# PINTO0309/human-instance-segmentation

Hardware: AMD Instinct MI355X
Metric: ROI-masks/sec (fwd) + train step/s, B0 640×480×8-ROI, 1/2/4/8 MI355X (higher is better)
Workload: dtype bf16; 1 GPU; C2: B0 inference 640x480, batch 32/GPU x 8 ROIs/img, ROI 64x48, mask 128x96; global_batch=32, parallelism=dp1 (images sharded, model replicated, no collective), schedule=2-stream pipeline (UNet of step k+1 overlaps head of step k)

## Files before the change

human-instance-segmentation_amd/csrc/conv_common.h:

```cpp
#pragma once
#include "common.h"

namespace hiseg {

typedef __bf16 bf16x8_t __attribute__((ext_vector_type(8)));
typedef float floatx4 __attribute__((ext_vector_type(4)));

struct ConvArgs {
  hiseg_conv2d_desc d;
  int M;
  int Cin;
  int nK;
  int Hs, Ws;
  int kper;
  int ins_vec;
  float* ws;
  int abl = 0;
};

int conv_fast_try(const ConvArgs& a, hipStream_t s, int variant);
int conv_wide_try(const ConvArgs& a, hipStream_t s, int variant);
int conv_hw_try(const ConvArgs& a, hipStream_t s, int variant);
int conv_hwr_try(const ConvArgs& a, hipStream_t s, int variant);
int conv_hwt_try(const ConvArgs& a, hipStream_t s, int variant);
int conv_hwc_try(const ConvArgs& a, hipStream_t s, int variant);
int conv_pw_try(const ConvArgs& a, hipStream_t s, int variant);
int conv_small_try(const ConvArgs& a, hipStream_t s, int variant);
int conv_rows_try(const ConvArgs& a, hipStream_t s, int variant);
bool conv_pw_applies(const ConvArgs& a);
int conv_pw_gate_images(const ConvArgs& a);
bool conv_rows_form(const ConvArgs& a);
int conv_hwc_stats_tiles(const ConvArgs& a);
int conv_hwc_fused_variant(const ConvArgs& a, bool r3);
int conv_generic_launch(const ConvArgs& a, hipStream_t s, int splits, int* bco);
int splitk_plan(const ConvArgs& a);
long long splitk_bytes(const ConvArgs& a, int splits);

template <typename T>
__device__ __forceinline__ void load4(const void* base, long long idx, bool vec, int nvalid,
                                      float* v) {
  if (vec) {
    if constexpr (sizeof(T) == 4) {
      float4 q = *reinterpret_cast<const float4*>(reinterpret_cast<const float*>(base) + idx);
      v[0] = q.x; v[1] = q.y; v[2] = q.z; v[3] = q.w;
    } else {
      uint2 q = *reinterpret_cast<const uint2*>(reinterpret_cast<const uint16_t*>(base) + idx);
      v[0] = __uint_as_float(q.x << 16); v[1] = __uint_as_float(q.x & 0xffff0000u);
      v[2] = __uint_as_float(q.y << 16); v[3] = __uint_as_float(q.y & 0xffff0000u);
    }
  } else {
#pragma unroll
    for (int e = 0; e < 4; ++e) v[e] = (e < nvalid) ? Elem<T>::load(base, idx + e) : 0.f;
  }
}

template <typename T>
__device__ __forceinline__ void store4(void* base, long long idx, bool vec, int nvalid,
                                       const float* v) {
  if (vec) {
    if constexpr (sizeof(T) == 4) {
      *reinterpret_cast<float4*>(reinterpret_cast<float*>(base) + idx) =
          make_float4(v[0], v[1], v[2], v[3]);
    } else {
      uint2 q;
      q.x = f2bf2(v[0], v[1]);
      q.y = f2bf2(v[2], v[3]);
      *reinterpret_cast<uint2*>(reinterpret_cast<uint16_t*>(base) + idx) = q;
    }
  } else {
#pragma unroll
    for (int e = 0; e < 4; ++e)
      if (e < nvalid) Elem<T>::store(base, idx + e, v[e]);
  }
}

__device__ __forceinline__ int swz(int row, int c) { return row * 8 + (c ^ ((row >> 1) & 7)); }

__device__ __forceinline__ void out_site(const hiseg_conv2d_desc& d, int px, int co, long long& op, int& oc) {
  if (d.convT) {
    const int Cq = d.Cout >> 2;
    const int q = co / Cq;
    oc = co - q * Cq;
    const int x = px % d.Wo;
    const int t = px / d.Wo;
    const int y = t % d.Ho;
    const int n = t / d.Ho;
// ... 148 lines not shown
```

human-instance-segmentation_amd/csrc/conv_dispatch.cpp:

```cpp
#include <atomic>
#include <climits>
#include <cstdlib>
#include "conv_common.h"

using namespace hiseg;

static std::atomic<long long> g_conv_paths[HISEG_CONV_PATH_FAMILIES];
static thread_local int g_conv_last = -1;

static void conv_note_path(int family, int variant) {
  g_conv_paths[family].fetch_add(1);
  g_conv_last = family * 10000 + variant;
}

extern "C" int hiseg_conv2d_last_path(void) { return g_conv_last; }

extern "C" int hiseg_conv2d_path_stats(long long* counts, int n, int reset) {
  for (int i = 0; i < HISEG_CONV_PATH_FAMILIES; ++i) {
    const long long c = reset ? g_conv_paths[i].exchange(0) : g_conv_paths[i].load();
    if (counts && i < n) counts[i] = c;
  }
  return HISEG_CONV_PATH_FAMILIES;
}

// ... 240 lines not shown
  return HISEG_OK;
}

static int conv2d_impl(const hiseg_conv2d_desc* d, hiseg_stream_t stream, int variant) {
  HISEG_REQUIRE(d != nullptr, HISEG_ERR_BAD_ARG, "conv2d: null descriptor");
  HISEG_REQUIRE(d->dtype == HISEG_F32 || d->dtype == HISEG_BF16, HISEG_ERR_BAD_DTYPE, "conv2d: dtype %d", d->dtype);
  HISEG_REQUIRE(d->out_dtype == HISEG_F32 || d->out_dtype == HISEG_BF16, HISEG_ERR_BAD_DTYPE, "conv2d: out_dtype %d", d->out_dtype);
  HISEG_REQUIRE(d->srcA && d->weight && d->scale && d->shift && (d->out || d->head2_out), HISEG_ERR_BAD_ARG,
                "conv2d: null pointer");
#ifdef HISEG_DIAG
  const bool fused_variant = variant == 0 || (variant == 148 && d->a_gate);
#else
  const bool fused_variant = variant == 0;
#endif
  HISEG_REQUIRE(!has_fused_operands(d) ||
                    (fused_variant && !d->stats_partial && !d->bnb_partial && fused_operands_ok(d)),
                HISEG_ERR_BAD_ARG,
                "conv2d: px_scale / head2_out / a_gate / res_gate go with the automatic choice alone: px_scale or "
                "a_gate by itself, res_gate only beside head2_out");
  HISEG_REQUIRE(d->N > 0 && d->H > 0 && d->W > 0 && d->Ho > 0 && d->Wo > 0, HISEG_ERR_BAD_SHAPE, "conv2d: empty grid");
  HISEG_REQUIRE(d->KH > 0 && d->KW > 0 && d->stride > 0 && d->pad >= 0, HISEG_ERR_BAD_SHAPE, "conv2d: bad window");
  HISEG_REQUIRE(d->a_up == 1 || d->a_up == 2, HISEG_ERR_BAD_SHAPE, "conv2d: a_up must be 1 or 2");
  HISEG_REQUIRE(d->a_up == 1 || (d->H % 2 == 0 && d->W % 2 == 0), HISEG_ERR_BAD_SHAPE, "conv2d: upsampled grid must be even");
  HISEG_REQUIRE(d->Cb == 0 || d->srcB, HISEG_ERR_BAD_ARG, "conv2d: Cb > 0 needs srcB");
  HISEG_REQUIRE(d->Cout > 0 && d->Cout_pad >= d->Cout && d->Cout_pad % 16 == 0, HISEG_ERR_BAD_SHAPE,
                "conv2d: Cout %d Cout_pad %d (must be multiple of 16)", d->Cout, d->Cout_pad);
  const int kch = d->dtype == HISEG_BF16 ? 8 : 4;
  const int bk = 8 * kch;
  const int Cin = d->Ca + d->Cb;
  HISEG_REQUIRE(d->Ca > 0 && d->Ca % kch == 0 && d->Cb % kch == 0 && d->a_cstride % kch == 0 &&
                    d->a_coff % kch == 0 && (d->Cb == 0 || (d->b_cstride % kch == 0 && d->b_coff % kch == 0)),
                HISEG_ERR_BAD_SHAPE, "conv2d: input channels/strides must be multiples of %d", kch);
  HISEG_REQUIRE(d->K_pad % bk == 0 && d->K_pad >= d->KH * d->KW * Cin, HISEG_ERR_BAD_SHAPE,
                "conv2d: K_pad %d must be a multiple of %d and >= %d", d->K_pad, bk, d->KH * d->KW * Cin);
  HISEG_REQUIRE(al16(d->srcA) && al16(d->srcB) && al16(d->weight), HISEG_ERR_BAD_SHAPE, "conv2d: operands must be 16-B aligned");
  HISEG_REQUIRE(!d->convT || (d->KH == 1 && d->KW == 1 && d->stride == 1 && d->pad == 0 && d->Cout % 16 == 0 &&
                              d->Ho == d->H && d->Wo == d->W),
                HISEG_ERR_BAD_SHAPE, "conv2d: convT requires a 1x1 GEMM with Cout = 4*C, C %% 4 == 0");
  hipStream_t s = (hipStream_t)stream;
  if (d->stats_partial || d->bnb_partial) {
    HISEG_REQUIRE(variant == 0 || variant == 104 || variant == 107, HISEG_ERR_BAD_ARG,
                  "conv2d: stats_partial / bnb_partial with variant %d", variant);
    HISEG_REQUIRE(al16(d->out) && al16(d->scale) && al16(d->shift), HISEG_ERR_BAD_SHAPE, "conv2d: alignment");
    const ConvArgs a = conv_args(*d);
    HISEG_REQUIRE(conv_hwc_stats_tiles(a) > 0, HISEG_ERR_BAD_ARG,
                  "conv2d: stats_partial / bnb_partial set but the layer has no fused kernel (hiseg_conv2d_stats_tiles)");
    const int r = conv_take({&kFamilies[F_HWC], d->Cout % 128 == 0 ? 104 : 107}, a, s);
    HISEG_REQUIRE(r != 0, HISEG_ERR_BAD_ARG, "conv2d: the fused-statistics kernel declined the layer");
    return r < 0 ? r : HISEG_OK;
  }
  return conv_in_ranges(d, s, variant);
}

extern "C" int hiseg_conv2d_fwd(const hiseg_conv2d_desc* d, hiseg_stream_t stream) {
  return conv2d_impl(d, stream, 0);
}

extern "C" int hiseg_conv2d_fwd_variant(const hiseg_conv2d_desc* d, int variant, hiseg_stream_t stream) {
#ifndef HISEG_DIAG
  HISEG_REQUIRE(release_variant(variant), HISEG_ERR_BAD_ARG,
                "conv2d: variant %d is not a release variant (diagnostic kernels need a DIAG=1 build)", variant);
#endif
  return conv2d_impl(d, stream, variant);
}
```

human-instance-segmentation_amd/hiseg/_lib.py:

```python
from __future__ import annotations

import contextlib
import ctypes
import os

import torch

_HERE = os.path.dirname(os.path.abspath(__file__))
LIB_PATH = os.environ.get("HISEG_LIB", os.path.join(_HERE, "libhiseg.so"))

HISEG_F32 = 0
HISEG_BF16 = 1
HISEG_POST_F32, HISEG_POST_F16, HISEG_POST_F32_TO_F16 = 0, 2, 3
ACT_NONE, ACT_RELU, ACT_SIGMOID, ACT_SILU, ACT_GELU, ACT_SWISH = 0, 1, 2, 3, 4, 5


class ActCode(int):

    def __new__(cls, code: int, beta: float = 1.0):
        o = int.__new__(cls, code)
        o.beta = float(beta)
        return o

    def __repr__(self):
# ... 200 lines not shown

class GuidedPrepDesc(Desc):
    _fields_ = [("mask", c_void_p), ("mask_stride", c_ll), ("N", c_int), ("h", c_int), ("w", c_int), ("dtype", c_int),
                ("fgp_c", c_void_p), ("fgp_cstride", c_int), ("fgp_coff", c_int),
                ("fg_prob", c_void_p), ("factor", c_void_p)]


class GuidedAttnDesc(Desc):
    _fields_ = [("dtype", c_int), ("x", c_void_p), ("P", c_ll), ("C", c_int), ("hidden", c_int),
                ("w1t", c_void_p), ("b1", c_void_p), ("w2", c_void_p), ("b2", c_void_p),
                ("act", c_int), ("act_beta", c_float),
                ("factor", c_void_p), ("att", c_void_p), ("gate", c_void_p), ("w1_frag", c_void_p)]


class GuidedFinishDesc(Desc):
    _fields_ = [("dtype", c_int), ("z", c_void_p), ("N", c_int), ("h", c_int), ("w", c_int), ("C", c_int),
                ("w3", c_void_p), ("b3", c_void_p), ("mh", c_int), ("mw", c_int), ("logits", c_void_p),
                ("mask", c_void_p), ("mask_stride", c_ll),
                ("bg_fg_logits", c_void_p), ("fg_prob", c_void_p), ("mask_out", c_void_p), ("tn_logits", c_void_p)]


class HisegError(RuntimeError):
    """Raised when a libhiseg entry point returns a non-zero status."""


_lib = None
_load_error = None


def _declare(lib):
    P = c_void_p
    sigs = {
        "hiseg_version": ([], c_int),
        "hiseg_last_error_string": ([], ctypes.c_char_p),
        "hiseg_built_for_gfx950": ([], c_int),
        "hiseg_stream_create_cu_mask": ([ctypes.POINTER(ctypes.c_uint), c_int, ctypes.POINTER(c_void_p)], c_int),
        "hiseg_stream_destroy": ([P], c_int),
        "hiseg_comm_load": ([ctypes.c_char_p], c_int),
        "hiseg_comm_unique_id": ([P], c_int),
        "hiseg_comm_init": ([ctypes.POINTER(c_void_p), c_int, P, c_int, c_int], c_int),
        "hiseg_comm_all_reduce": ([P, P, c_ll, c_int, c_int, P], c_int),
        "hiseg_comm_destroy": ([P], c_int),
        "hiseg_roi_align_fwd": ([ctypes.POINTER(RoiAlignDesc), P], c_int),
        "hiseg_conv2d_fwd": ([ctypes.POINTER(Conv2dDesc), P], c_int),
        "hiseg_conv2d_fwd_variant": ([ctypes.POINTER(Conv2dDesc), c_int, P], c_int),
        "hiseg_conv2d_workspace_bytes": ([ctypes.POINTER(Conv2dDesc)], c_ll),
        "hiseg_conv2d_last_path": ([], c_int),
        "hiseg_conv2d_path_stats": ([ctypes.POINTER(c_ll), c_int, c_int], c_int),
        "hiseg_maxpool2x2_fwd": ([c_int, P, c_int, c_int, c_int, c_int, P, P], c_int),
        "hiseg_attn_spatial_fwd": ([c_int, P, c_int, c_int, c_int, c_int, P, c_int, P, P, P, P], c_int),
        "hiseg_attn_map_fwd": ([c_int, P, c_int, c_int, c_int, c_int, P, c_int, P, P, P], c_int),
        "hiseg_pixel_scale_fwd": ([c_int, P, c_ll, c_int, P, P, P], c_int),
        "hiseg_conv2d_fused_ok": ([ctypes.POINTER(Conv2dDesc)], c_int),
        "hiseg_hier_combine_tn_fwd": ([P, c_int, c_int, c_int, P, P, P, P, c_int, c_float, c_int, P, P, P, P, P, P],
                                      c_int),
        "hiseg_gap_splits": ([c_int], c_int),
        "hiseg_se_gate_fwd": ([c_int, P, c_int, c_int, c_int, P, P, c_int, P, P, c_int, c_float, P, P, P], c_int),
        "hiseg_channel_scale_fwd": ([c_int, P, c_int, c_int, c_int, P, P, P], c_int),
        "hiseg_dwconv_fwd": ([c_int, P, c_int, c_int, c_int, c_int, c_int, c_int, P, P, P, c_int, P,
                              c_int, c_int, P], c_int),
        "hiseg_dw_gap_tiles": ([c_int, c_int, c_int], c_int),
        "hiseg_dw_gap_parts": ([c_int, c_int, c_int, c_int, c_int, c_int, c_int], c_int),
        "hiseg_dwconv_gap_fwd": ([c_int, P, c_int, c_int, c_int, c_int, c_int, c_int, P, P, P, c_int, P,
                                  c_int, c_int, P, P], c_int),
        "hiseg_se_gate_partials_fwd": ([P, c_int, c_int, c_int, c_int, P, P, c_int, P, P, c_int, P, P], c_int),
        "hiseg_image_max_fwd": ([P, c_ll, P, P], c_int),
        "hiseg_input_norm_fwd": ([c_int, P, c_int, c_int, c_int, c_int, P, P, P, P, c_int, P], c_int),
        "hiseg_hier_combine_fwd": ([c_int, P, c_int, c_int, c_int, P, c_int, P, P, P, c_int, c_float, c_int, P, P,
                                    P, P, P, P, P, P], c_int),
        "hiseg_ubf_ln_tables": ([P, c_int, c_int, c_int, P, P, P, P, c_float, c_int, P, P, P, P, P], c_int),
        "hiseg_nhwc_to_nchw_fwd": ([c_int, P, c_int, c_int, c_int, c_int, c_int, c_int, P, P], c_int),
        "hiseg_nchw_to_nhwc_fwd": ([c_int, P, c_int, c_int, c_int, c_int, P, c_int, P], c_int),
        "hiseg_instance_masks_fwd": ([P, c_int, c_int, c_int, c_int, P, P], c_int),
        "hiseg_binary_masks_fwd": ([c_int, P, c_int, c_int, c_int, c_int, P, P, P, P], c_int),
        "hiseg_resize_bilinear_fwd": ([P, c_int, c_int, c_int, P, c_int, c_int, P], c_int),
        "hiseg_distance_mask_fwd": ([P, c_ll, P, P, P], c_int),
        "hiseg_output_conv_fwd": ([P, c_int, c_int, c_int, P, P, P, P], c_int),
        "hiseg_conv2d_wgrad_dims": ([ctypes.POINTER(Conv2dDesc), c_int, P, P, P], c_int),
        "hiseg_conv2d_wgrad": ([ctypes.POINTER(Conv2dDesc), P, c_int, c_int, c_int, P, c_int, P], c_int),
        "hiseg_wgrad_path_stats": ([ctypes.POINTER(c_ll), c_int], c_int),
        "hiseg_struct_sizes": ([ctypes.POINTER(c_ll), c_int], c_int),
        "hiseg_conv2d_stats_tiles": ([ctypes.POINTER(Conv2dDesc)], c_int),
        "hiseg_bn_finalize_n": ([P, c_int, c_int, c_ll, P, P, c_float, c_float, P, P, P, P, P, P, P], c_int),
        "hiseg_wgrad_last_path": ([], c_int),
        "hiseg_conv2d_wgrad_reduce": ([P, c_int, ctypes.POINTER(WgradMap), P, P, c_int, P], c_int),
        "hiseg_pack_weights": ([P, c_int, c_int, P], c_int),
        "hiseg_bn_partials": ([], c_int),
        "hiseg_bn_last_path": ([], c_int),
        "hiseg_bn_stats": ([c_int, P, c_ll, c_int, c_int, c_int, P, P], c_int),
        "hiseg_bn_finalize": ([P, c_int, c_ll, P, P, c_float, c_float, P, P, P, P, P, P, P], c_int),
        "hiseg_bn_apply": ([ctypes.POINTER(BnApplyDesc), P], c_int),
        "hiseg_bn_bwd": ([ctypes.POINTER(BnBwdDesc), P], c_int),
        "hiseg_dropout2d_mask": ([c_int, c_int, c_float, ctypes.c_ulonglong, P, P], c_int),
        "hiseg_dropout2d_mask_dev": ([c_int, c_int, c_float, P, ctypes.c_ulonglong, P, P], c_int),
        "hiseg_seed_advance": ([P, P], c_int),
        "hiseg_relu_bwd": ([c_int, c_ll, c_int, c_int, EwView, EwView, P, EwView, P], c_int),
        "hiseg_sigmoid_bwd": ([c_int, c_ll, c_int, EwView, EwView, EwView, P], c_int),
        "hiseg_gate_fwd": ([c_int, c_ll, c_int, EwView, EwView, EwView, P], c_int),
        "hiseg_gate_bwd": ([c_int, c_ll, c_int, EwView, EwView, EwView, EwView, c_int, EwView, P], c_int),
        "hiseg_add_inplace": ([c_int, c_ll, c_int, EwView, EwView, P], c_int),
        "hiseg_act_bwd_cvt": ([c_int, c_ll, c_int, EwView, EwView, c_int, EwView, c_int, P], c_int),
        "hiseg_act_bwd_pre": ([c_int, c_ll, c_int, EwView, EwView, c_int, c_float, EwView, c_int, P], c_int),
        "hiseg_ln_ws": ([c_int, c_int, c_int], c_ll),
        "hiseg_ln_fwd_stats": ([c_int, P, c_int, c_int, c_int, c_int, c_int, P, P, c_float, P, P, P, P, P, P],
                               c_int),
        "hiseg_ln_bwd": ([ctypes.POINTER(LnBwdDesc), P], c_int),
# ... 127 lines not shown
        handle = ctypes.CDLL(LIB_PATH, mode=ctypes.RTLD_GLOBAL)
        EXPORTED = list(_declare(handle))
    except OSError as e:
        _load_error = ImportError(f"failed to load {LIB_PATH}: {e}")
        raise _load_error
    if handle.hiseg_built_for_gfx950() != 1:
        _load_error = ImportError("libhiseg.so was not built for gfx950")
        raise _load_error
    _lib = handle
    return _lib


def check(status: int, what: str) -> None:
    if status != 0:
        msg = lib().hiseg_last_error_string().decode(errors="replace")
        raise HisegError(f"{what} failed with status {status}: {msg}")


def placement_stats(reset: bool = False):
    a, b = c_ll(), c_ll()
    check(lib().hiseg_placement_stats(ctypes.byref(a), ctypes.byref(b), int(reset)), "placement_stats")
    return a.value, b.value


WGRAD_PATHS = ("wide", "transposed_read", "generic_bf16", "f32", "halo")


def wgrad_path_stats(reset: bool = False) -> dict:
    c = (c_ll * 5)()
    check(lib().hiseg_wgrad_path_stats(c, int(reset)), "wgrad_path_stats")
    return dict(zip(WGRAD_PATHS, (int(v) for v in c)))


def wgrad_last_path():
    v = lib().hiseg_wgrad_last_path()
    return None if v < 0 else WGRAD_PATHS[v]


BN_ENTRIES = ("stats", "finalize", "apply", "bwd")
BN_BWD_MODES = ("none", "y", "relu_pre", "pre")


def bn_path_decode(v: int):
    if v < 0:
        return None
    return {"entry": BN_ENTRIES[v & 3], "vec": bool(v & 4), "par": bool(v & 8), "premerge": bool(v & 16),
            "mode": BN_BWD_MODES[(v >> 5) & 3], "reduce": bool(v & 128), "u2": bool(v & 256)}


def bn_last_path():
    return bn_path_decode(lib().hiseg_bn_last_path())


CONV_PATHS = ("generic", "generic_splitk", "fast", "wide", "hw", "hwr", "hwt", "hwc", "pw", "small", "rows")


def conv_last_path():
    v = lib().hiseg_conv2d_last_path()
    return None if v < 0 else (CONV_PATHS[v // 10000], v % 10000)


def conv_path_stats(reset: bool = False) -> dict:
    c = (c_ll * len(CONV_PATHS))()
    n = lib().hiseg_conv2d_path_stats(c, len(CONV_PATHS), int(reset))
    assert n == len(CONV_PATHS), n
    return dict(zip(CONV_PATHS, (int(v) for v in c)))


def stream_ptr(device=None) -> int:
    return torch.cuda.current_stream(device).cuda_stream
```

human-instance-segmentation_amd/hiseg/engine.py:

```python
from __future__ import annotations

from typing import Dict, Optional, Tuple

import torch
import torch.nn as nn

from . import _lib as L
from . import ops
from .effunet import DepthwiseSeparableConv, InvertedResidual
from .layers import LayerNorm2d, Swish
from .ops import Act, round_up

ACT_NONE, ACT_RELU, ACT_SIGMOID, ACT_SILU = L.ACT_NONE, L.ACT_RELU, L.ACT_SIGMOID, L.ACT_SILU
ACT_GELU, ACT_SWISH = L.ACT_GELU, L.ACT_SWISH


def act_code(m: nn.Module) -> int:
    if isinstance(m, nn.ReLU):
        return ACT_RELU
    if isinstance(m, nn.SiLU):
        return ACT_SILU
    if isinstance(m, Swish):
        return ACT_SILU if float(m.beta) == 1.0 else L.ActCode(ACT_SWISH, float(m.beta))
    if isinstance(m, nn.GELU):
# ... 52 lines not shown

    def conv(self, conv: nn.Conv2d, bn=None, act: int = ACT_NONE, split=None) -> ops.ConvPlan:
        def build():
            assert conv.groups == 1 and conv.dilation in ((1, 1), 1)
            assert conv.kernel_size[0] == conv.kernel_size[1] and conv.stride[0] == conv.stride[1]
            return ops.pack_conv(conv.weight, conv.bias, _bn(bn), act, self.dtype, self.device,
                                 stride=conv.stride[0], pad=conv.padding[0], split=split)
        return self._get(("conv", id(conv), act, split), build, (conv.weight, conv.bias) + _bn_tensors(bn))

    def convT(self, conv: nn.ConvTranspose2d, bn=None, act: int = ACT_NONE) -> ops.ConvPlan:
        def build():
            assert conv.kernel_size == (2, 2) and conv.stride == (2, 2) and conv.padding == (0, 0)
            return ops.pack_convT2x2(conv.weight, conv.bias, _bn(bn), act, self.dtype, self.device)
        return self._get(("convT", id(conv), act), build, (conv.weight, conv.bias) + _bn_tensors(bn))

    def f32(self, t: torch.Tensor, shape=None) -> torch.Tensor:
        def build():
            v = t.detach().to(device=self.device, dtype=torch.float32).contiguous()
            return v.view(shape) if shape is not None else v
        return self._get(("f32", id(t), shape), build, (t,))

    def affine(self, key, cout, bias, bn):
        def build():
            s, h = ops.fold_affine(cout, bias, _bn(bn), self.device)
            return s.contiguous(), h.contiguous()
        return self._get(("aff", key), build, (bias,) + _bn_tensors(bn))

    def dw(self, conv: nn.Conv2d, bn):
        def build():
            c, _, k, _ = conv.weight.shape
            w = conv.weight.detach().float().to(self.device).view(c, k * k).t().contiguous()
            s, h = ops.fold_affine(c, conv.bias, _bn(bn), self.device)
            return w, s.contiguous(), h.contiguous(), k, conv.stride[0]
        return self._get(("dw", id(conv)), build, (conv.weight, conv.bias) + _bn_tensors(bn))


def cna(E: Ctx, conv: nn.Module, norm: Optional[nn.Module], act: int, x: Act, xb: Optional[Act] = None, *,
        split=None, residual: Optional[Act] = None, out: Optional[Act] = None, convT: bool = False) -> Act:
    if isinstance(norm, LayerNorm2d):
        plan = E.convT(conv, None, ACT_NONE) if convT else E.conv(conv, None, ACT_NONE, split=split)
        z = ops.conv2d(plan, x, xb)
        C = z.C
        return ops.layernorm2d(z, E.f32(norm.weight, (C,)), E.f32(norm.bias, (C,)), norm.eps, act,
                               residual=residual, out=out)
    plan = E.convT(conv, norm, act) if convT else E.conv(conv, norm, act, split=split)
    return ops.conv2d(plan, x, xb, residual=residual, out=out)


def _check_input(x: torch.Tensor, what: str):
    if not x.is_cuda:
        raise RuntimeError(f"{what}: hiseg runs on the GPU only (got a CPU tensor); there is no CPU fallback")


def _block_acts(blk: nn.Module) -> Tuple[int, int]:
    return (act_code(blk.activation1 if hasattr(blk, "activation1") else blk.activation),
            act_code(blk.activation2 if hasattr(blk, "activation2") else blk.activation))


def gated_block_ok(E: Ctx, blk: nn.Module, x: Act, gate: torch.Tensor, head2: ops.Head2) -> bool:
    if isinstance(blk.norm1, LayerNorm2d) or isinstance(blk.norm2, LayerNorm2d) or x.dtype != torch.bfloat16:
        return False
    a1, a2 = _block_acts(blk)
    p1, p2 = E.conv(blk.conv1, blk.norm1, a1), E.conv(blk.conv2, blk.norm2, a2)
    if p1.cout != x.C or p2.cout != x.C:
        return False
    return ops._fused_ok(p1, x, None, None, None, None, None, None, x.dtype, 1, a_gate=gate) and \
        ops._fused_ok(p2, x, None, x, None, None, None, head2, x.dtype, 1, res_gate=gate)


def residual_block(E: Ctx, blk: nn.Module, x: Act, out: Optional[Act] = None,
                   head2: Optional[ops.Head2] = None, in_gate: Optional[torch.Tensor] = None) -> Optional[Act]:
    a1, a2 = _block_acts(blk)
    if in_gate is not None:
        h = ops.conv2d(E.conv(blk.conv1, blk.norm1, a1), x, a_gate=in_gate)
        return ops.conv2d(E.conv(blk.conv2, blk.norm2, a2), h, residual=x, res_gate=in_gate, head2=head2)
    h = cna(E, blk.conv1, blk.norm1, a1, x)
    if head2 is not None and out is None and not isinstance(blk.norm2, LayerNorm2d):
        return ops.conv2d(E.conv(blk.conv2, blk.norm2, a2), h, residual=x, head2=head2)
    return cna(E, blk.conv2, blk.norm2, a2, h, residual=x, out=out)


def rgb_feature_extractor(E: Ctx, seq: nn.Sequential, x: Act, out: Optional[Act] = None) -> Act:
    h = cna(E, seq[0], seq[1], act_code(seq[2]), x)
    h = residual_block(E, seq[3], h)
    h = cna(E, seq[4], seq[5], act_code(seq[6]), h)
    h = residual_block(E, seq[7], h)
    h = cna(E, seq[8], seq[9], act_code(seq[10]), h)
    h = residual_block(E, seq[11], h)
    return cna(E, seq[12], seq[13], act_code(seq[14]), h, out=out)


def enhanced_unet(E: Ctx, u: nn.Module, x: Act) -> Tuple[Act, Act]:
    d = u.depth
    if x.H % (1 << (d - 1)) or x.W % (1 << (d - 1)):
        raise NotImplementedError(
            f"ROI size {x.H}x{x.W} is not divisible by 2^{d - 1}: the reference's bilinear resize of the up-conv "
            "output (unet.py:408) is then not the identity; not supported on the hiseg path")
    feats = []
    for i in range(d):
        enc = u.encoders[i]
        if i == 0:
            x = cna(E, enc[0], enc[1], act_code(enc[2]), x)
            x = residual_block(E, enc[3], x)
            x = residual_block(E, enc[4], x)
        else:
            x = residual_block(E, enc[0], x)
            x = residual_block(E, enc[1], x)
            x = cna(E, enc[2], enc[3], act_code(enc[4]), x)
        feats.append(x)
        if i < d - 1:
            x = ops.maxpool2x2(x)
    b = u.bottleneck
    a = residual_block(E, b[0], x)
    a = residual_block(E, b[1], a)
    a = cna(E, b[2], b[3], act_code(b[4]), a)
    att = ops.conv2d(E.conv(b[5], None, ACT_SIGMOID), a)
    x = ops.conv2d(E.conv(u.bottleneck_conv), x, mul=att)
    for i in range(d - 1):
        up = ops.conv2d(E.convT(u.upconvs[i]), x)
        skip = feats[d - 2 - i]
        dec = u.decoders[i]
        x = cna(E, dec[0], dec[1], act_code(dec[2]), up, skip, split=(up.C, skip.C))
        x = residual_block(E, dec[3], x)
        x = residual_block(E, dec[4], x)
    f = u.final
# ... 449 lines not shown
```

human-instance-segmentation_amd/hiseg/ops.py:

```python
from __future__ import annotations

import ctypes
from dataclasses import dataclass
from typing import Optional

import torch

from . import _lib as L

_TORCH_TO_HISEG = {torch.float32: L.HISEG_F32, torch.bfloat16: L.HISEG_BF16}


def chunk_elems(dtype: torch.dtype) -> int:
    return 8 if dtype == torch.bfloat16 else 4


def round_up(x: int, m: int) -> int:
    return (x + m - 1) // m * m


def hdtype(dtype: torch.dtype) -> int:
    try:
        return _TORCH_TO_HISEG[dtype]
    except KeyError:
# ... 312 lines not shown
    if residual is not None:
        d.residual, d.r_cstride, d.r_coff = residual, residual.cstride, residual.coff
    if mul is not None:
        d.mul, d.m_cstride, d.m_coff = mul, mul.cstride, mul.coff
    if out is not None:
        d.out, d.o_cstride, d.o_coff = out, out.cstride, out.coff
    else:
        d.o_cstride, d.o_coff = p.cout, 0
    if head2 is not None:
        d.head2_w, d.head2_b, d.head2_out = head2.w, head2.b, head2_out
    if px_scale is not None:
        d.px_scale = px_scale
    if a_gate is not None:
        d.a_gate = a_gate
    if res_gate is not None:
        d.res_gate = res_gate
    if out2 is not None:
        assert out2.dtype == dt
        d.out2, d.o2_cstride, d.o2_coff = out2, out2.cstride, out2.coff
    d.convT = int(p.convT)
    if p.weight_frag is not None:
        d.weight_frag = p.weight_frag
    return d


def _conv_flops(d, p, xa, xb) -> float:
    return 2.0 * d.N * d.Ho * d.Wo * p.gemm_cols * p.kh * p.kw * (xa.C + (xb.C if xb is not None else 0))


def _fused_ok(p, xa, xb, residual, mul, in_scale, px_scale, head2, out_dtype, a_up, a_gate=None, res_gate=None) -> bool:
    if xa.dtype != torch.bfloat16 or out_dtype != torch.bfloat16 or xb is not None or mul is not None or \
            in_scale is not None or a_up != 1:
        return False
    for gt, c in ((a_gate, p.ca), (res_gate, p.cout)):
        if gt is not None:
            assert gt.dtype == torch.float32 and gt.is_contiguous() and tuple(gt.shape) == (xa.N, c), \
                (gt.dtype, tuple(gt.shape), (xa.N, c))
    if a_gate is not None and xa.C != p.ca:
        return False
    if px_scale is not None:
        assert px_scale.dtype == torch.float32 and px_scale.is_contiguous() and px_scale.numel() == xa.N * xa.H * xa.W
    if head2 is not None:
        if p.convT or residual is None:
            return False
        assert head2.w.dtype == torch.float32 and head2.w.is_contiguous() and tuple(head2.w.shape) == (2, p.cout)
        assert head2.b.dtype == torch.float32 and head2.b.numel() == 2
    d = _conv_desc(p, xa, None, residual, None, None, out_dtype=out_dtype, px_scale=px_scale, head2=head2,
                   head2_out=head2.w if head2 is not None else None, a_gate=a_gate, res_gate=res_gate)
    if px_scale is not None or a_gate is not None:
        d.out = xa
    return bool(L.lib().hiseg_conv2d_fused_ok(ctypes.byref(d)))


def _launch_conv(d, p, xa, xb, variant=0):
    if PROBE is not None:
        key = PROBE.select(d)
        if key is not None:
            L.check(PROBE.around(key, _conv_flops(d, p, xa, xb), lambda: L.lib().hiseg_conv2d_fwd(ctypes.byref(d), L.stream_ptr())),
                    "conv2d")
            return
    if variant:
        L.check(L.lib().hiseg_conv2d_fwd_variant(ctypes.byref(d), variant, L.stream_ptr()), "conv2d")
    else:
        L.check(L.lib().hiseg_conv2d_fwd(ctypes.byref(d), L.stream_ptr()), "conv2d")


def maxpool2x2(x: Act) -> Act:
    assert x.coff == 0 and x.cstride == x.cpad
    out = Act.new(x.N, x.H // 2, x.W // 2, x.C, x.dtype, x.t.device, cpad=x.cstride, zero=False)
    L.check(L.lib().hiseg_maxpool2x2_fwd(hdtype(x.dtype), x.ptr(), x.N, x.H, x.W, x.cstride, out.ptr(),
                                         L.stream_ptr()), "maxpool2x2")
    return out


def attn_spatial(x: Act, w7: torch.Tensor) -> Act:
    assert x.coff == 0 and x.cstride == x.C
    P = x.N * x.H * x.W
    stats = torch.empty(P * 2, dtype=torch.float32, device=x.t.device)
    att = torch.empty(P, dtype=torch.float32, device=x.t.device)
    out = Act.new(x.N, x.H, x.W, x.C, x.dtype, x.t.device, zero=False)
    k = w7.shape[-1]
    L.check(L.lib().hiseg_attn_spatial_fwd(hdtype(x.dtype), x.ptr(), x.N, x.H, x.W, x.C, w7.data_ptr(), k,
                                           stats.data_ptr(), att.data_ptr(), out.ptr(), L.stream_ptr()),
            "attn_spatial")
    return out


def attn_map(x: Act, w7: torch.Tensor) -> torch.Tensor:
    assert x.coff == 0 and x.cstride == x.C
    P = x.N * x.H * x.W
    stats = torch.empty(P * 2, dtype=torch.float32, device=x.t.device)
    att = torch.empty(P, dtype=torch.float32, device=x.t.device)
    L.check(L.lib().hiseg_attn_map_fwd(hdtype(x.dtype), x.ptr(), x.N, x.H, x.W, x.C, w7.data_ptr(), w7.shape[-1],
                                       stats.data_ptr(), att.data_ptr(), L.stream_ptr()), "attn_map")
    return att


def pixel_scale(x: Act, att: torch.Tensor) -> Act:
    assert x.coff == 0 and x.cstride == x.C and att.dtype == torch.float32 and att.numel() == x.N * x.H * x.W
    out = Act.new(x.N, x.H, x.W, x.C, x.dtype, x.t.device, zero=False)
    L.check(L.lib().hiseg_pixel_scale_fwd(hdtype(x.dtype), x.ptr(), x.N * x.H * x.W, x.C, att.data_ptr(), out.ptr(),
                                          L.stream_ptr()), "pixel_scale")
    return out


def se_gate(x: Act, w1, b1, w2, b2, act: int) -> torch.Tensor:
# ... 606 lines not shown
```

include/hiseg.h:

```cpp
#ifndef HISEG_H_
#define HISEG_H_

#ifdef __cplusplus
extern "C" {
#endif

typedef void* hiseg_stream_t;

enum hiseg_dtype { HISEG_F32 = 0, HISEG_BF16 = 1 };

enum hiseg_act { HISEG_ACT_NONE = 0, HISEG_ACT_RELU = 1, HISEG_ACT_SIGMOID = 2, HISEG_ACT_SILU = 3,
                 HISEG_ACT_GELU = 4, HISEG_ACT_SWISH = 5 };

enum hiseg_status {
  HISEG_OK = 0,
  HISEG_ERR_BAD_ARG = -1,
  HISEG_ERR_BAD_SHAPE = -2,
  HISEG_ERR_BAD_DTYPE = -3,
  HISEG_ERR_LAUNCH = -4
};

int hiseg_version(void);
const char* hiseg_last_error_string(void);
int hiseg_built_for_gfx950(void);
int hiseg_debug_fill_lds(unsigned pattern, int rounds, hiseg_stream_t stream);
int hiseg_placement_stats(long long* declined, long long* far, int reset);

int hiseg_stream_create_cu_mask(const unsigned* mask, int nwords, hiseg_stream_t* out);
int hiseg_stream_destroy(hiseg_stream_t s);

typedef struct hiseg_roi_align_desc {
  const float* feat; int B, C, H, W;
  const float* rois; int N;
  int oh, ow;
  float scale_h, scale_w;
  int aligned;
  const float* aff_w; const float* aff_b; int n_aff;
  void* out; int out_dtype; int o_cstride; int o_coff; int o_nchw; int zero_to;
} hiseg_roi_align_desc;
int hiseg_roi_align_fwd(const hiseg_roi_align_desc* d, hiseg_stream_t stream);

typedef struct hiseg_conv2d_desc {
  int dtype, out_dtype;
  int N, H, W;
  int Ho, Wo;
  int KH, KW, stride, pad;
  const void* srcA; int a_cstride, a_coff, Ca, a_up;
  const void* srcB; int b_cstride, b_coff, Cb;
  const float* in_scale;
  const void* weight; int Cout, Cout_pad, K_pad;
  const float* scale; const float* shift;
  int act;
  const void* residual; int r_cstride, r_coff;
  const void* mul; int m_cstride, m_coff;
  void* out; int o_cstride, o_coff;
  void* out2; int o2_cstride, o2_coff;
  int convT;
  const void* weight_frag;
  float act_beta;
  void* workspace; long long workspace_bytes;
  float* stats_partial;
  float* bnb_partial; const void* bnb_z; int bnb_z_cstride, bnb_z_coff;
  const float* bnb_scale; const float* bnb_shift; const float* bnb_mean; const float* bnb_invstd; int bnb_act;
  const float* px_scale;
  const float* head2_w; const float* head2_b; float* head2_out;
  const float* a_gate; const float* res_gate;
} hiseg_conv2d_desc;
int hiseg_conv2d_fwd(const hiseg_conv2d_desc* d, hiseg_stream_t stream);
int hiseg_conv2d_fused_ok(const hiseg_conv2d_desc* d);
int hiseg_struct_sizes(long long* out, int n);
long long hiseg_conv2d_workspace_bytes(const hiseg_conv2d_desc* d);
int hiseg_conv2d_stats_tiles(const hiseg_conv2d_desc* d);
int hiseg_conv2d_fwd_variant(const hiseg_conv2d_desc* d, int variant, hiseg_stream_t stream);
#define HISEG_CONV_PATH_GENERIC 0
#define HISEG_CONV_PATH_GENERIC_SPLITK 1
#define HISEG_CONV_PATH_FAST 2
#define HISEG_CONV_PATH_WIDE 3
#define HISEG_CONV_PATH_HW 4
#define HISEG_CONV_PATH_HWR 5
#define HISEG_CONV_PATH_HWT 6
#define HISEG_CONV_PATH_HWC 7
#define HISEG_CONV_PATH_PW 8
#define HISEG_CONV_PATH_SMALL 9
#define HISEG_CONV_PATH_ROWS 10
#define HISEG_CONV_PATH_FAMILIES 11
int hiseg_conv2d_last_path(void);
int hiseg_conv2d_path_stats(long long* counts, int n, int reset);

int hiseg_maxpool2x2_fwd(int dtype, const void* in, int N, int H, int W, int C, void* out,
                         hiseg_stream_t stream);

int hiseg_attn_spatial_fwd(int dtype, const void* x, int N, int H, int W, int C, const float* w7,
                           int k, float* stats, float* att, void* out, hiseg_stream_t stream);
int hiseg_attn_map_fwd(int dtype, const void* x, int N, int H, int W, int C, const float* w7,
                       int k, float* stats, float* att, hiseg_stream_t stream);
int hiseg_pixel_scale_fwd(int dtype, const void* x, long long P, int C, const float* att, void* out,
                          hiseg_stream_t stream);

int hiseg_gap_splits(int HW);
int hiseg_se_gate_fwd(int dtype, const void* x, int N, int HW, int C, const float* w1,
                      const float* b1, int Cr, const float* w2, const float* b2, int act, float act_beta,
                      float* partial, float* gate, hiseg_stream_t stream);

int hiseg_channel_scale_fwd(int dtype, const void* x, int N, int HW, int C, const float* gate,
                            void* out, hiseg_stream_t stream);

int hiseg_dwconv_fwd(int dtype, const void* in, int N, int H, int W, int C, int K, int stride,
                     const float* w, const float* scale, const float* shift, int act, void* out,
                     int Ho, int Wo, hiseg_stream_t stream);
int hiseg_dw_gap_tiles(int N, int Ho, int Wo);
int hiseg_dw_gap_parts(int dtype, int N, int Ho, int Wo, int C, int K, int stride);
int hiseg_dwconv_gap_fwd(int dtype, const void* in, int N, int H, int W, int C, int K, int stride,
                         const float* w, const float* scale, const float* shift, int act, void* out,
                         int Ho, int Wo, float* gap_partial, hiseg_stream_t stream);
int hiseg_se_gate_partials_fwd(float* partial, int splits, int N, int HW, int C, const float* w1,
                               const float* b1, int Cr, const float* w2, const float* b2, int act,
                               float* gate, hiseg_stream_t stream);

int hiseg_image_max_fwd(const float* x, long long n, float* maxbuf, hiseg_stream_t stream);
int hiseg_input_norm_fwd(int dtype, const float* x, int B, int C, int H, int W, const float* maxbuf,
                         const float* mean, const float* std, void* out, int cpad,
                         hiseg_stream_t stream);

int hiseg_hier_combine_fwd(int dtype, const float* low, int N, int h, int w, const void* tfeat,
                           int Ct, const float* ut_w, const float* ut_scale, const float* ut_shift,
                           int ut_act, float ut_beta, int ut_per_sample, const float* u1_w,
                           const float* u1_b, const float* t_w, const float* t_b, float* logits,
                           float* bgfg, float* tn, hiseg_stream_t stream);
int hiseg_hier_combine_tn_fwd(const float* low, int N, int h, int w, const float* tn2, const float* ut_w,
                              const float* ut_scale, const float* ut_shift, int ut_act, float ut_beta,
                              int ut_per_sample, const float* u1_w, const float* u1_b, float* logits,
                              float* bgfg, float* tn, hiseg_stream_t stream);
int hiseg_ubf_ln_tables(const float* low, int N, int h, int w, const float* ut_w, const float* ut_b,
                        const float* gamma, const float* beta, float eps, int fold_bias, float* mean,
                        float* invstd, float* scale, float* shift, hiseg_stream_t stream);

int hiseg_nhwc_to_nchw_fwd(int dtype, const void* in, int N, int H, int W, int C, int cstride,
                           int coff, float* out, hiseg_stream_t stream);
// ... 23 lines not shown
```

Before: 16590 ROI-masks/s.

## Fuse residual block's two 3x3 convs into one tiled LDS-resident kernel

```diff
diff --git a/human-instance-segmentation_amd/csrc/conv_common.h b/human-instance-segmentation_amd/csrc/conv_common.h
--- a/human-instance-segmentation_amd/csrc/conv_common.h
+++ b/human-instance-segmentation_amd/csrc/conv_common.h
@@ -32,6 +32,8 @@
 bool conv_rows_form(const ConvArgs& a);
 int conv_hwc_stats_tiles(const ConvArgs& a);
 int conv_hwc_fused_variant(const ConvArgs& a, bool r3);
+bool conv_resblock_applies(const hiseg_conv2d_desc& d1, const hiseg_conv2d_desc& d2);
+int conv_resblock_launch(const hiseg_conv2d_desc& d1, const hiseg_conv2d_desc& d2, hipStream_t s);
 int conv_generic_launch(const ConvArgs& a, hipStream_t s, int splits, int* bco);
 int splitk_plan(const ConvArgs& a);
 long long splitk_bytes(const ConvArgs& a, int splits);
diff --git a/human-instance-segmentation_amd/csrc/conv_dispatch.cpp b/human-instance-segmentation_amd/csrc/conv_dispatch.cpp
--- a/human-instance-segmentation_amd/csrc/conv_dispatch.cpp
+++ b/human-instance-segmentation_amd/csrc/conv_dispatch.cpp
@@ -316,6 +316,19 @@
   return conv_in_ranges(d, s, variant);
 }
 
+extern "C" int hiseg_resblock_fused_ok(const hiseg_conv2d_desc* d1, const hiseg_conv2d_desc* d2) {
+  return d1 != nullptr && d2 != nullptr && conv_resblock_applies(*d1, *d2) ? 1 : 0;
+}
+
+extern "C" int hiseg_resblock_fwd(const hiseg_conv2d_desc* d1, const hiseg_conv2d_desc* d2, hiseg_stream_t stream) {
+  HISEG_REQUIRE(d1 != nullptr && d2 != nullptr, HISEG_ERR_BAD_ARG, "resblock: null descriptor");
+  HISEG_REQUIRE(conv_resblock_applies(*d1, *d2), HISEG_ERR_BAD_ARG,
+                "resblock: the pair of layers has no fused kernel (hiseg_resblock_fused_ok)");
+  const int r = conv_resblock_launch(*d1, *d2, (hipStream_t)stream);
+  if (r == HISEG_OK) conv_note_path(HISEG_CONV_PATH_RESBLOCK, 1);
+  return r;
+}
+
 extern "C" int hiseg_conv2d_fwd(const hiseg_conv2d_desc* d, hiseg_stream_t stream) {
   return conv2d_impl(d, stream, 0);
 }
diff --git a/human-instance-segmentation_amd/csrc/conv_resblock.hip b/human-instance-segmentation_amd/csrc/conv_resblock.hip
--- /dev/null
+++ b/human-instance-segmentation_amd/csrc/conv_resblock.hip
@@ -0,0 +1,354 @@
+#include "conv_common.h"
+
+namespace hiseg {
+
+typedef unsigned rb_u4 __attribute__((ext_vector_type(4)));
+typedef __attribute__((address_space(3))) void rb_lds_void;
+
+__device__ __forceinline__ void rb_dma16(__amdgpu_buffer_rsrc_t rsrc, unsigned lds_addr, unsigned voff) {
+  asm volatile("s_mov_b32 m0, %0\n\ts_nop 0\n\tbuffer_load_dwordx4 %1, %2, 0 offen lds"
+               :: "s"(__builtin_amdgcn_readfirstlane(lds_addr)), "v"(voff), "s"(rsrc) : "memory");
+}
+
+constexpr int RB_HP = 20;
+constexpr int RB_NPI = 26;
+constexpr int RB_PLANE_I = RB_NPI * 1024;
+constexpr int RB_NF = 23;
+constexpr int RB_PLANE_M = RB_NF * 1024;
+constexpr int RB_LDS = 2 * RB_PLANE_I;
+
+template <int ACT1, int ACT2>
+__global__ void __launch_bounds__(256, 2) conv_resblock_kernel(hiseg_conv2d_desc d1, hiseg_conv2d_desc d2) {
+  constexpr int NW = 4, FPW = 12, NR2 = 8;
+  extern __shared__ __attribute__((aligned(16))) uint4 smem[];
+  const int t = threadIdx.x;
+  const int lane = t & 63;
+  const int w = __builtin_amdgcn_readfirstlane(t >> 6);
+  const int wc = w & 1, ph = w >> 1;
+
+  const int ntx = (d1.W + 15) >> 4, nty = (d1.H + 15) >> 4;
+  const int nwg = gridDim.x;
+  const int orig = blockIdx.x;
+  const int q8 = nwg >> 3, r8 = nwg & 7, xcd = orig & 7, loc = orig >> 3;
+  int tl = (xcd < r8 ? xcd * (q8 + 1) : r8 * (q8 + 1) + (xcd - r8) * q8) + loc;
+  const int tx = tl % ntx;
+  tl /= ntx;
+  const int ty = tl % nty;
+  const int n = tl / nty;
+  const int y0 = ty * 16, x0 = tx * 16;
+  const int H = d1.H, W = d1.W;
+
+  const unsigned OOB = 0x80000000u;
+  const __amdgpu_buffer_rsrc_t rF1 = __builtin_amdgcn_make_buffer_rsrc(
+      const_cast<void*>(d1.weight_frag), (short)0, 64 * 9 * 64 * 2, 0x00020000);
+  const __amdgpu_buffer_rsrc_t rF2 = __builtin_amdgcn_make_buffer_rsrc(
+      const_cast<void*>(d2.weight_frag), (short)0, 64 * 9 * 64 * 2, 0x00020000);
+  const __amdgpu_buffer_rsrc_t rA = __builtin_amdgcn_make_buffer_rsrc(
+      const_cast<void*>(d1.srcA), (short)0, d1.N * H * W * d1.a_cstride * 2, 0x00020000);
+
+  auto load_blk = [&](rb_u4 (&af)[3][2], const __amdgpu_buffer_rsrc_t& rF, int sl, int kx) __attribute__((always_inline)) {
+    int ln = lane;
+    asm volatile("" : "+v"(ln));
+    const unsigned a_lane = (unsigned)(2 * wc) * 18u * 1024u + (unsigned)ln * 16u;
+#pragma unroll
+    for (int ky = 0; ky < 3; ++ky) {
+      const unsigned so = __builtin_amdgcn_readfirstlane(((unsigned)(ky * 3 + kx) * 2u + (unsigned)sl) * 1024u);
+#pragma unroll
+      for (int i = 0; i < 2; ++i)
+        af[ky][i] = __builtin_amdgcn_raw_buffer_load_b128(rF, a_lane + (unsigned)i * 18u * 1024u, so, 0);
+    }
+  };
+
+  const unsigned lds_base = (unsigned)(uintptr_t)(rb_lds_void*)smem;
+  const char* lds_c = reinterpret_cast<const char*>(smem);
+  char* lds_w = reinterpret_cast<char*>(smem);
+
+#pragma unroll
+  for (int k = 0; k < 13; ++k) {
+    const int g = w + NW * k;
+    const int sl = g >= RB_NPI ? 1 : 0, pc = g - RB_NPI * sl;
+    int ln = lane;
+    asm volatile("" : "+v"(ln));
+    const int p = 16 * pc + (ln >> 2);
+    const int hy = p / RB_HP, hx = p - RB_HP * hy;
+    const int iy = y0 - 2 + hy, ix = x0 - 2 + hx;
+    const bool ok = hy < RB_HP && (unsigned)iy < (unsigned)H && (unsigned)ix < (unsigned)W;
+    const int chunk = (ln & 3) ^ (((p >> 2) & 1) << 1);
+    const unsigned off =
+        ok ? (unsigned)((((n * H + iy) * W + ix) * d1.a_cstride + d1.a_coff + 32 * sl + chunk * 8) * 2) : OOB;
+    rb_dma16(rA, lds_base + (unsigned)(RB_PLANE_I * sl + 1024 * pc), off);
+  }
+  rb_u4 af[3][2], an[3][2];
+  load_blk(af, rF1, 0, 0);
+  asm volatile("s_waitcnt vmcnt(0)" ::: "memory");
+  __syncthreads();
+
+  const int j16 = lane & 15, c4 = lane >> 4;
+
+  floatx4 acc[2][FPW];
+#pragma unroll
+  for (int i = 0; i < 2; ++i)
+#pragma unroll
+    for (int k = 0; k < FPW; ++k) acc[i][k] = floatx4{0.f, 0.f, 0.f, 0.f};
+  const int klast = ph ? FPW - 2 : FPW - 1;
+  {
+    constexpr int RA = 4;
+    auto block1 = [&](int sl, auto kxc, bool last) __attribute__((always_inline)) {
+      constexpr int KX = decltype(kxc)::value;
+      if (!last) load_blk(an, rF1, KX < 2 ? sl : sl + 1, KX < 2 ? KX + 1 : 0);
+      else load_blk(an, rF2, 0, 0);
+      int ln = lane;
+      asm volatile("" : "+v"(ln));
+      const int j = ln & 15, cc = ln >> 4;
+      int adr[3];
+#pragma unroll
+      for (int ky = 0; ky < 3; ++ky) {
+        const int tt = j + RB_HP * ky + KX;
+        adr[ky] = RB_PLANE_I * sl + (16 * FPW * ph + tt) * 64 + ((cc ^ (((tt >> 2) & 1) << 1)) << 4);
+      }
+      auto rd = [&](int idx) __attribute__((always_inline)) -> rb_u4 {
+        const int ky = idx / FPW, k = idx % FPW;
+        const int ko = k == FPW - 1 ? klast * 1024 : k * 1024;
+        return *reinterpret_cast<const rb_u4*>(lds_c + adr[ky] + ko);
+      };
+      rb_u4 bq[RA + 1];
+#pragma unroll
+      for (int r = 0; r < RA; ++r) bq[r] = rd(r);
+      __builtin_amdgcn_s_setprio(1);
+#pragma unroll
+      for (int idx = 0; idx < 3 * FPW; ++idx) {
+        if (idx + RA < 3 * FPW) bq[(idx + RA) % (RA + 1)] = rd(idx + RA);
+        __builtin_amdgcn_sched_barrier(0);
+        const int ky = idx / FPW, k = idx % FPW;
+#pragma unroll
+        for (int i = 0; i < 2; ++i)
+          acc[i][k] = __builtin_amdgcn_mfma_f32_16x16x32_bf16(__builtin_bit_cast(bf16x8_t, af[ky][i]),
+                                                              __builtin_bit_cast(bf16x8_t, bq[idx % (RA + 1)]),
+                                                              acc[i][k], 0, 0, 0);
+      }
+      __builtin_amdgcn_s_setprio(0);
+#pragma unroll
+      for (int ky = 0; ky < 3; ++ky)
+#pragma unroll
+        for (int i = 0; i < 2; ++i) af[ky][i] = an[ky][i];
+    };
+    using K0 = std::integral_constant<int, 0>;
+    using K1 = std::integral_constant<int, 1>;
+    using K2 = std::integral_constant<int, 2>;
+    block1(0, K0{}, false);
+    block1(0, K1{}, false);
+    block1(0, K2{}, false);
+    block1(1, K0{}, false);
+    block1(1, K1{}, false);
+    block1(1, K2{}, true);
+  }
+  {
+    floatx4 sc[2], sh[2];
+#pragma unroll
+    for (int i = 0; i < 2; ++i) {
+      const int cl = wc * 32 + i * 16 + c4 * 4;
+      sc[i] = *reinterpret_cast<const floatx4*>(d1.scale + cl);
+      sh[i] = *reinterpret_cast<const floatx4*>(d1.shift + cl);
+    }
+    __syncthreads();
+#pragma unroll
+    for (int k = 0; k < FPW; ++k) {
+      if (k == FPW - 1 && ph) continue;
+      const int m = 16 * (FPW * ph + k) + j16;
+      const int iy = m / RB_HP, ix = m - RB_HP * iy;
+      const int gy = y0 - 1 + iy, gx = x0 - 1 + ix;
+      const bool ok = ix < 18 && iy < 18 && (unsigned)gy < (unsigned)H && (unsigned)gx < (unsigned)W;
+#pragma unroll
+      for (int i = 0; i < 2; ++i) {
+        const floatx4 ac = acc[i][k];
+        float v[4];
+#pragma unroll
+        for (int e = 0; e < 4; ++e) {
+          v[e] = ac[e] * sc[i][e] + sh[i][e];
+          if constexpr (ACT1 == HISEG_ACT_RELU) v[e] = v[e] > 0.f ? v[e] : 0.f;
+        }
+        uint2 o;
+        o.x = f2bf2(v[0], v[1]);
+        o.y = f2bf2(v[2], v[3]);
+        if (!ok) o = make_uint2(0u, 0u);
+        const int ch = 2 * i + (c4 >> 1);
+        *reinterpret_cast<uint2*>(lds_w + RB_PLANE_M * wc + m * 64 + ((ch ^ (((m >> 2) & 1) << 1)) << 4) +
+                                  ((c4 & 1) << 3)) = o;
+      }
+    }
+    __syncthreads();
+  }
+
+  floatx4 ac2[2][NR2];
+#pragma unroll
+  for (int i = 0; i < 2; ++i)
+#pragma unroll
+    for (int jr = 0; jr < NR2; ++jr) ac2[i][jr] = floatx4{0.f, 0.f, 0.f, 0.f};
+  {
+    auto block2 = [&](int sl, auto kxc, bool last) __attribute__((always_inline)) {
+      constexpr int KX = decltype(kxc)::value;
+      if (!last) load_blk(an, rF2, KX < 2 ? sl : sl + 1, KX < 2 ? KX + 1 : 0);
+      int ln = lane;
+      asm volatile("" : "+v"(ln));
+      const int j = ln & 15, cc = ln >> 4;
+      const int se = (cc ^ ((((KX + j) >> 2) & 1) << 1)) << 4;
+      const int base = RB_PLANE_M * sl + (NR2 * RB_HP * ph + KX + j) * 64;
+      auto rd = [&](int r) __attribute__((always_inline)) -> rb_u4 {
+        return *reinterpret_cast<const rb_u4*>(lds_c + base + ((r & 1) ? (se ^ 32) : se) + r * RB_HP * 64);
+      };
+      rb_u4 bq[3];
+      bq[0] = rd(0);
+      bq[1] = rd(1);
+      __builtin_amdgcn_s_setprio(1);
+#pragma unroll
+      for (int r = 0; r < NR2 + 2; ++r) {
+        if (r + 2 < NR2 + 2) bq[(r + 2) % 3] = rd(r + 2);
+        __builtin_amdgcn_sched_barrier(0);
+#pragma unroll
+        for (int ky = 0; ky < 3; ++ky) {
+          const int jr = r - ky;
+          if (jr >= 0 && jr < NR2) {
+#pragma unroll
+            for (int i = 0; i < 2; ++i)
+              ac2[i][jr] = __builtin_amdgcn_mfma_f32_16x16x32_bf16(__builtin_bit_cast(bf16x8_t, af[ky][i]),
+                                                                   __builtin_bit_cast(bf16x8_t, bq[r % 3]),
+                                                                   ac2[i][jr], 0, 0, 0);
+          }
+        }
+      }
+      __builtin_amdgcn_s_setprio(0);
+      if (!last) {
+#pragma unroll
+        for (int ky = 0; ky < 3; ++ky)
+#pragma unroll
+          for (int i = 0; i < 2; ++i) af[ky][i] = an[ky][i];
+      }
+    };
+    using K0 = std::integral_constant<int, 0>;
+    using K1 = std::integral_constant<int, 1>;
+    using K2 = std::integral_constant<int, 2>;
+    block2(0, K0{}, false);
+    block2(0, K1{}, false);
+    block2(0, K2{}, false);
+    block2(1, K0{}, false);
+    block2(1, K1{}, false);
+    block2(1, K2{}, true);
+  }
+  __syncthreads();
+
+  constexpr int EROWB = 128, CPR = 8, RPI = 8, SWM = 7, NRI = 256 / (RPI * NW), NST = 256 * CPR / (NW * 64);
+  auto px_of = [&](int r) __attribute__((always_inline)) -> int {
+    const int y = y0 + (r >> 4), x = x0 + (r & 15);
+    return (y < H && x < W) ? (n * H + y) * W + x : -1;
+  };
+  const __amdgpu_buffer_rsrc_t rR = __builtin_amdgcn_make_buffer_rsrc(
+      const_cast<void*>(d2.residual), (short)0, d1.N * H * W * d2.r_cstride * 2, 0x00020000);
+#pragma unroll
+  for (int k = 0; k < NRI; ++k) {
+    int ln = lane;
+    asm volatile("" : "+v"(ln));
+    const int c = ln % CPR;
+    const int r = RPI * (w + NW * k) + ln / CPR;
+    const int px = px_of(r);
+    const unsigned off = px >= 0 ? (unsigned)((px * d2.r_cstride + d2.r_coff + ((c ^ (r & SWM)) * 8)) * 2) : OOB;
+    rb_dma16(rR, lds_base + (unsigned)(RPI * (w + NW * k) * EROWB), off);
+  }
+  floatx4 sc[2], sh[2];
+#pragma unroll
+  for (int i = 0; i < 2; ++i) {
+    const int cl = wc * 32 + i * 16 + c4 * 4;
+    sc[i] = *reinterpret_cast<const floatx4*>(d2.scale + cl);
+    sh[i] = *reinterpret_cast<const floatx4*>(d2.shift + cl);
+  }
+  asm volatile("s_waitcnt vmcnt(0)" ::: "memory");
+  __syncthreads();
+  char* tile = lds_w;
+#pragma unroll
+  for (int i = 0; i < 2; ++i)
+#pragma unroll
+    for (int jr = 0; jr < NR2; ++jr) {
+      const int cl = wc * 32 + i * 16 + c4 * 4;
+      const int r = (NR2 * ph + jr) * 16 + j16;
+      char* q = tile + r * EROWB + ((((cl >> 3) ^ (r & SWM)) << 4) | ((cl & 4) << 1));
+      const floatx4 ac = ac2[i][jr];
+      float v[4];
+      const uint2 rv = *reinterpret_cast<const uint2*>(q);
+#pragma unroll
+      for (int e = 0; e < 4; ++e) {
+        v[e] = ac[e] * sc[i][e] + sh[i][e];
+        v[e] += Quad<bf16_t>::get(rv, e);
+        if constexpr (ACT2 == HISEG_ACT_RELU) v[e] = v[e] > 0.f ? v[e] : 0.f;
+      }
+      uint2 o;
+      o.x = f2bf2(v[0], v[1]);
+      o.y = f2bf2(v[2], v[3]);
+      *reinterpret_cast<uint2*>(q) = o;
+    }
+  __syncthreads();
+  uint4 sv[NST];
+#pragma unroll
+  for (int k = 0; k < NST; ++k) {
+    const int idx = t + NW * 64 * k;
+    const int r = idx / CPR, c = idx % CPR;
+    sv[k] = *reinterpret_cast<const uint4*>(tile + r * EROWB + ((c ^ (r & SWM)) << 4));
+  }
+  const __amdgpu_buffer_rsrc_t rO = __builtin_amdgcn_make_buffer_rsrc(
+      d2.out, (short)0, d1.N * H * W * d2.o_cstride * 2, 0x00020000);
+#pragma unroll
+  for (int k = 0; k < NST; ++k) {
+    const int idx = t + NW * 64 * k;
+    const int r = idx / CPR, c = idx % CPR;
+    const int px = px_of(r);
+    __builtin_amdgcn_raw_buffer_store_b128(__builtin_bit_cast(rb_u4, sv[k]), rO,
+                                           px >= 0 ? (unsigned)((px * d2.o_cstride + d2.o_coff + 8 * c) * 2) : OOB, 0, 0);
+  }
+}
+
+bool conv_resblock_applies(const hiseg_conv2d_desc& d1, const hiseg_conv2d_desc& d2) {
+  for (const hiseg_conv2d_desc* d : {&d1, &d2}) {
+    if (d->dtype != HISEG_BF16 || d->out_dtype != HISEG_BF16 || d->weight_frag == nullptr) return false;
+    if (d->KH != 3 || d->KW != 3 || d->stride != 1 || d->pad != 1 || d->convT || d->a_up != 1) return false;
+    if (d->Ca != 64 || d->Cb != 0 || d->srcB || d->Cout != 64 || d->Cout_pad != 64 || d->K_pad != 576) return false;
+    if (d->act != HISEG_ACT_NONE && d->act != HISEG_ACT_RELU) return false;
+    if (d->in_scale || d->mul || d->out2 || d->stats_partial || d->bnb_partial || d->px_scale || d->head2_out ||
+        d->head2_w || d->a_gate || d->res_gate || d->workspace)
+      return false;
+    if (!d->scale || !d->shift || (((uintptr_t)d->scale | (uintptr_t)d->shift | (uintptr_t)d->weight_frag) & 15))
+      return false;
+    if (d->N != d1.N || d->H != d1.H || d->W != d1.W || d->Ho != d1.H || d->Wo != d1.W) return false;
+  }
+  if (d1.N <= 0 || d1.H <= 0 || d1.W <= 0) return false;
+  if (d1.residual || !d1.srcA || ((uintptr_t)d1.srcA & 15) || ((d1.a_cstride | d1.a_coff) & 7) || d1.a_cstride < 64)
+    return false;
+  if (d2.residual != d1.srcA || d2.r_cstride != d1.a_cstride || d2.r_coff != d1.a_coff) return false;
+  if (!d2.out || ((uintptr_t)d2.out & 15) || d2.o_cstride != 64 || d2.o_coff != 0) return false;
+  const long long px = (long long)d1.N * d1.H * d1.W;
+  if (px * d1.a_cstride * 2 >= 0x7fffffffll || px * d2.o_cstride * 2 >= 0x7fffffffll) return false;
+  const long long tiles = (long long)d1.N * ((d1.H + 15) / 16) * ((d1.W + 15) / 16);
+  if (tiles >= (1ll << 31)) return false;
+  if (d2.out == d1.srcA) return false;
+  return true;
+}
+
+template <int ACT1, int ACT2>
+static int launch_resblock(const hiseg_conv2d_desc& d1, const hiseg_conv2d_desc& d2, hipStream_t s) {
+  auto kern = conv_resblock_kernel<ACT1, ACT2>;
+  static bool attr = false;
+  if (!attr) {
+    (void)hipFuncSetAttribute((const void*)kern, hipFuncAttributeMaxDynamicSharedMemorySize, RB_LDS);
+    attr = true;
+  }
+  const int tiles = d1.N * ((d1.H + 15) / 16) * ((d1.W + 15) / 16);
+  hipLaunchKernelGGL(kern, dim3(tiles), dim3(256), RB_LDS, s, d1, d2);
+  return hiseg_check_launch("conv_resblock");
+}
+
+int conv_resblock_launch(const hiseg_conv2d_desc& d1, const hiseg_conv2d_desc& d2, hipStream_t s) {
+  const bool r1 = d1.act == HISEG_ACT_RELU, r2 = d2.act == HISEG_ACT_RELU;
+  return r1 ? (r2 ? launch_resblock<HISEG_ACT_RELU, HISEG_ACT_RELU>(d1, d2, s)
+                  : launch_resblock<HISEG_ACT_RELU, HISEG_ACT_NONE>(d1, d2, s))
+            : (r2 ? launch_resblock<HISEG_ACT_NONE, HISEG_ACT_RELU>(d1, d2, s)
+                  : launch_resblock<HISEG_ACT_NONE, HISEG_ACT_NONE>(d1, d2, s));
+}
+
+}
diff --git a/human-instance-segmentation_amd/hiseg/_lib.py b/human-instance-segmentation_amd/hiseg/_lib.py
--- a/human-instance-segmentation_amd/hiseg/_lib.py
+++ b/human-instance-segmentation_amd/hiseg/_lib.py
@@ -276,6 +276,8 @@
         "hiseg_attn_map_fwd": ([c_int, P, c_int, c_int, c_int, c_int, P, c_int, P, P, P], c_int),
         "hiseg_pixel_scale_fwd": ([c_int, P, c_ll, c_int, P, P, P], c_int),
         "hiseg_conv2d_fused_ok": ([ctypes.POINTER(Conv2dDesc)], c_int),
+        "hiseg_resblock_fused_ok": ([ctypes.POINTER(Conv2dDesc), ctypes.POINTER(Conv2dDesc)], c_int),
+        "hiseg_resblock_fwd": ([ctypes.POINTER(Conv2dDesc), ctypes.POINTER(Conv2dDesc), P], c_int),
         "hiseg_hier_combine_tn_fwd": ([P, c_int, c_int, c_int, P, P, P, P, c_int, c_float, c_int, P, P, P, P, P, P],
                                       c_int),
         "hiseg_gap_splits": ([c_int], c_int),
@@ -509,7 +511,7 @@
     return bn_path_decode(lib().hiseg_bn_last_path())
 
 
-CONV_PATHS = ("generic", "generic_splitk", "fast", "wide", "hw", "hwr", "hwt", "hwc", "pw", "small", "rows")
+CONV_PATHS = ("generic", "generic_splitk", "fast", "wide", "hw", "hwr", "hwt", "hwc", "pw", "small", "rows", "resblock")
 
 
 def conv_last_path():
diff --git a/human-instance-segmentation_amd/hiseg/engine.py b/human-instance-segmentation_amd/hiseg/engine.py
--- a/human-instance-segmentation_amd/hiseg/engine.py
+++ b/human-instance-segmentation_amd/hiseg/engine.py
@@ -128,6 +128,9 @@
         raise RuntimeError(f"{what}: hiseg runs on the GPU only (got a CPU tensor); there is no CPU fallback")
 
 
+RESBLOCK_FUSED = True
+
+
 def _block_acts(blk: nn.Module) -> Tuple[int, int]:
     return (act_code(blk.activation1 if hasattr(blk, "activation1") else blk.activation),
             act_code(blk.activation2 if hasattr(blk, "activation2") else blk.activation))
@@ -147,6 +150,12 @@
 def residual_block(E: Ctx, blk: nn.Module, x: Act, out: Optional[Act] = None,
                    head2: Optional[ops.Head2] = None, in_gate: Optional[torch.Tensor] = None) -> Optional[Act]:
     a1, a2 = _block_acts(blk)
+    if RESBLOCK_FUSED and in_gate is None and head2 is None and out is None and x.C == 64 and \
+            x.dtype == torch.bfloat16 and not isinstance(blk.norm1, LayerNorm2d) and \
+            not isinstance(blk.norm2, LayerNorm2d):
+        y = ops.resblock(E.conv(blk.conv1, blk.norm1, a1), E.conv(blk.conv2, blk.norm2, a2), x)
+        if y is not None:
+            return y
     if in_gate is not None:
         h = ops.conv2d(E.conv(blk.conv1, blk.norm1, a1), x, a_gate=in_gate)
         return ops.conv2d(E.conv(blk.conv2, blk.norm2, a2), h, residual=x, res_gate=in_gate, head2=head2)
diff --git a/human-instance-segmentation_amd/hiseg/ops.py b/human-instance-segmentation_amd/hiseg/ops.py
--- a/human-instance-segmentation_amd/hiseg/ops.py
+++ b/human-instance-segmentation_amd/hiseg/ops.py
@@ -388,6 +388,19 @@
     return bool(L.lib().hiseg_conv2d_fused_ok(ctypes.byref(d)))
 
 
+def resblock(p1: ConvPlan, p2: ConvPlan, x: Act) -> Optional[Act]:
+    if RECORD is not None or GATE is not None or x.dtype != torch.bfloat16 or p1.convT or p2.convT or \
+            p1.cout != 64 or p2.cout != 64 or x.C != 64:
+        return None
+    out = Act.new(x.N, x.H, x.W, p2.cout, x.dtype, x.t.device, zero=None)
+    d1 = _conv_desc(p1, x, None, None, None, None, out_dtype=x.dtype)
+    d2 = _conv_desc(p2, x, None, x, None, out)
+    if not L.lib().hiseg_resblock_fused_ok(ctypes.byref(d1), ctypes.byref(d2)):
+        return None
+    L.check(L.lib().hiseg_resblock_fwd(ctypes.byref(d1), ctypes.byref(d2), L.stream_ptr()), "resblock")
+    return out
+
+
 def _launch_conv(d, p, xa, xb, variant=0):
     if PROBE is not None:
         key = PROBE.select(d)
diff --git a/include/hiseg.h b/include/hiseg.h
--- a/include/hiseg.h
+++ b/include/hiseg.h
@@ -68,6 +68,8 @@
 } hiseg_conv2d_desc;
 int hiseg_conv2d_fwd(const hiseg_conv2d_desc* d, hiseg_stream_t stream);
 int hiseg_conv2d_fused_ok(const hiseg_conv2d_desc* d);
+int hiseg_resblock_fused_ok(const hiseg_conv2d_desc* d1, const hiseg_conv2d_desc* d2);
+int hiseg_resblock_fwd(const hiseg_conv2d_desc* d1, const hiseg_conv2d_desc* d2, hiseg_stream_t stream);
 int hiseg_struct_sizes(long long* out, int n);
 long long hiseg_conv2d_workspace_bytes(const hiseg_conv2d_desc* d);
 int hiseg_conv2d_stats_tiles(const hiseg_conv2d_desc* d);
@@ -83,7 +85,8 @@
 #define HISEG_CONV_PATH_PW 8
 #define HISEG_CONV_PATH_SMALL 9
 #define HISEG_CONV_PATH_ROWS 10
-#define HISEG_CONV_PATH_FAMILIES 11
+#define HISEG_CONV_PATH_RESBLOCK 11
+#define HISEG_CONV_PATH_FAMILIES 12
 int hiseg_conv2d_last_path(void);
 int hiseg_conv2d_path_stats(long long* counts, int n, int reset);
 
```

After: 16880 ROI-masks/s (median of 6 runs). 1.8% higher.
